# AshHarvey/ssa-gym

Measured on AMD Instinct MI355X. Metric: env_steps_per_sec_at_20k_objects, higher is better.
Workload: dtype f64

## Files before the change

### ssa-gym_amd/csrc/ssa_kernels.hip

```cpp
#include <hip/hip_runtime.h>
#include <cstdio>
#include <cstddef>
#include <cstdlib>
#include <hip/hip_ext.h>
#include <stdint.h>
#include <type_traits>

#include "../../include/ssa_hip.h"
#include "ssa_math.hpp"
#include "ssa_conics.hpp"
#include "ssa_screen.hpp"

namespace ssa {

__device__ __noinline__ Vec6 kepler_general_v(Vec6 x, double tof)
{
    Vec6 o;
    kepler_general_impl(x.v, tof, o.v, nullptr);
    return o;
}
template <int TAG>
__device__ __noinline__ Vec6 kepler_general_tagged(Vec6 x, double tof)
{
    Vec6 o;
// ... 225 lines not shown
        v = sqrt_fast(t.P[g * 36 + 7 * off] + t.P[g * 36 + 7 * (off + 1)] + t.P[g * 36 + 7 * (off + 2)]);
    }
    return v;
}
SSA_DEV void observe_rows(Tiles& t, int g, int l, bool stage_obs)
{
    if (stage_obs && l < 12) t.Obs[g * 12 + l] = (l < 6) ? t.X[g * 6 + l] : t.P[g * 36 + 7 * (l - 6)];
    if (l < 4) t.Met[g * 4 + l] = metric_value(t, g, l);
}

struct Moments { double c00, c01, c11; };
template <bool SUMS_ONLY = false>
SSA_DEV Moments moment_sums_mfma(Tiles& t, int lane)
{
    const int hi = lane >> 4, mid = (lane >> 2) & 3, lo = lane & 3;
    const double* src = &t.D[dbase(mid) + hi * 8 + lo];
    double a0[3], a1[3];
#pragma unroll
    for (int kc = 0; kc < 3; ++kc) {
        a0[kc] = src[kc * 32];
        a1[kc] = src[kc * 32 + 4];
    }
    Moments mo = {0.0, 0.0, 0.0};
#pragma unroll
    for (int kc = 0; kc < 3; ++kc) {
        if (!SUMS_ONLY) mo.c00 = __builtin_amdgcn_mfma_f64_4x4x4f64(a0[kc], a0[kc], mo.c00, 0, 0, 0);
        mo.c01 = __builtin_amdgcn_mfma_f64_4x4x4f64(a0[kc], a1[kc], mo.c01, 0, 0, 0);
        mo.c11 = __builtin_amdgcn_mfma_f64_4x4x4f64(a1[kc], a1[kc], mo.c11, 0, 0, 0);
    }
    if (lo == 2) {
        t.M[mid * 12 + hi] = mo.c01;
        if (hi < 2) t.M[mid * 12 + 4 + hi] = mo.c11;
    }
    return mo;
}

SSA_DEV double covariance_entry(const ssa_consts& C, double acc, double sa_, double ma, double sb_, double mb, double q)
{
    return C.Wi * acc - ma * sb_ - sa_ * mb + C.sum_wc * ma * mb + q;
}
SSA_DEV void covariance_finish(Tiles& t, const ssa_consts& C, int lane, const Moments& mo)
{
    const int hi = lane >> 4, mid = (lane >> 2) & 3, lo = lane & 3;
    const int hi1 = hi & 1, lo1 = lo & 1;
    const double* M = &t.M[mid * 12];
    double* P = &t.P[mid * 36];
    const double s_a = M[hi], m_a = M[6 + hi], s_b = M[lo], m_b = M[6 + lo];
    const double s_a4 = M[4 + hi1], m_a4 = M[10 + hi1], s_b4 = M[4 + lo1], m_b4 = M[10 + lo1];
    const double p00 = covariance_entry(C, mo.c00, s_a, m_a, s_b, m_b, t.Q[hi * 6 + lo]);
    const double p01 = covariance_entry(C, mo.c01, s_a, m_a, s_b4, m_b4, t.Q[hi * 6 + 4 + lo1]);
    const double p11 = covariance_entry(C, mo.c11, s_a4, m_a4, s_b4, m_b4, t.Q[(4 + hi1) * 6 + 4 + lo1]);
    if (hi <= lo) {
        P[hi * 6 + lo] = p00;
        P[lo * 6 + hi] = p00;
    }
    if (lo < 2) {
        P[hi * 6 + 4 + lo] = p01;
        P[(4 + lo) * 6 + hi] = p01;
        if (hi <= lo) {
            P[(4 + hi) * 6 + 4 + lo] = p11;
            P[(4 + lo) * 6 + 4 + hi] = p11;
        }
    }
}

struct StatAcc {
    double mx, sm;
    long long arg;
    unsigned c4, c7, nf;
    int mx_nan, sm_nan;
};
SSA_DEV void stat_merge(StatAcc& a, const StatAcc& b)
{
    a.mx = fmax(a.mx, b.mx);
    a.mx_nan |= b.mx_nan;
    a.c4 += b.c4; a.c7 += b.c7; a.nf += b.nf;
    bool take_b;
    if (a.sm_nan || b.sm_nan) take_b = b.sm_nan && (!a.sm_nan || b.arg < a.arg);
    else take_b = (b.sm > a.sm) || (b.sm == a.sm && b.arg < a.arg);
    if (take_b) { a.sm = b.sm; a.arg = b.arg; a.sm_nan = b.sm_nan; }
}
SSA_DEV StatAcc stat_shfl_down(const StatAcc& a, int off)
{
    StatAcc b;
    b.mx = __shfl_down(a.mx, off, 64);
    b.sm = __shfl_down(a.sm, off, 64);
    b.arg = __shfl_down(a.arg, off, 64);
    b.c4 = __shfl_down(a.c4, off, 64);
    b.c7 = __shfl_down(a.c7, off, 64);
    b.nf = __shfl_down(a.nf, off, 64);
    b.mx_nan = __shfl_down(a.mx_nan, off, 64);
    b.sm_nan = __shfl_down(a.sm_nan, off, 64);
    return b;
}
SSA_DEV StatAcc stat_identity()
{
    StatAcc a;
    a.mx = -1.0; a.sm = -1.0; a.arg = 0x7fffffffffffffffLL; a.c4 = a.c7 = a.nf = 0; a.mx_nan = a.sm_nan = 0;
    return a;
}
SSA_DEV StatAcc stat_wave_reduce(StatAcc a)
{
#pragma unroll
    for (int off = 32; off > 0; off >>= 1) {
        StatAcc b = stat_shfl_down(a, off);
        stat_merge(a, b);
    }
    return a;
}

SSA_DEV void wave_lds_sync()
{
    __builtin_amdgcn_fence(__ATOMIC_ACQ_REL, "wavefront");
    __builtin_amdgcn_wave_barrier();
    asm volatile("" ::: "memory");
}

SSA_DEV int ybase(int g) { return g * 104 + (g & 1) * 28 + (g >> 1) * 32; }
SSA_DEV void covariance_reference(Tiles& t, const ssa_consts& C, int lane, const double (&o)[6], double xb_l)
{
    static_assert(372 + 16 * 8 <= OBJ_PER_WAVE * 36 + 408, "y rows fit the factor tile + D");
    typedef double v2d_t __attribute__((ext_vector_type(2)));
    double* const Y = t.UA;
    {
        const int g = lane >> 4, l = lane & 15;
        const double x0 = row_bcast<0>(xb_l), x1 = row_bcast<1>(xb_l), x2 = row_bcast<2>(xb_l), x3 = row_bcast<3>(xb_l),
                     x4 = row_bcast<4>(xb_l), x5 = row_bcast<5>(xb_l);
        if (l <= 12) {
            v2d_t* dst = reinterpret_cast<v2d_t*>(&Y[ybase(g) + l * 8]);
            dst[0] = v2d_t{o[0] - x0, o[1] - x1};
            dst[1] = v2d_t{o[2] - x2, o[3] - x3};
            dst[2] = v2d_t{o[4] - x4, o[5] - x5};
            dst[3] = v2d_t{0.0, 0.0};
        }
    }
    wave_lds_sync();
    const int hi = lane >> 4, mid = (lane >> 2) & 3, lo = lane & 3;
    const double* src = &Y[ybase(mid) + hi * 8 + lo];
    Moments mo = {0.0, 0.0, 0.0};
    constexpr int NKC = 3;
#pragma unroll
    for (int kc = 0; kc < NKC; ++kc) {
        double a0 = src[kc * 32], a1 = src[kc * 32 + 4];
        if (kc == 3 && hi != 0) { a0 = 0.0; a1 = 0.0; }
        const double w = (kc == 0 && hi == 0) ? C.Wc0 : C.Wi;
        const double b0 = w * a0, b1 = w * a1;
        mo.c00 = __builtin_amdgcn_mfma_f64_4x4x4f64(a0, b0, mo.c00, 0, 0, 0);
        mo.c01 = __builtin_amdgcn_mfma_f64_4x4x4f64(a0, b1, mo.c01, 0, 0, 0);
        mo.c11 = __builtin_amdgcn_mfma_f64_4x4x4f64(a1, b1, mo.c11, 0, 0, 0);
    }
    {
        const double* y12 = &Y[ybase(mid) + 12 * 8];
        const double ai = y12[hi], ai4 = y12[4 + hi], bj = C.Wi * y12[lo], bj4 = C.Wi * y12[4 + lo];
        mo.c00 = fma(ai, bj, mo.c00);
        mo.c01 = fma(ai, bj4, mo.c01);
        mo.c11 = fma(ai4, bj4, mo.c11);
    }
    const int hi1 = hi & 1, lo1 = lo & 1;
    double* P = &t.P[mid * 36];
    const double p00 = mo.c00 + t.Q[hi * 6 + lo];
    const double p01 = mo.c01 + t.Q[hi * 6 + 4 + lo1];
    const double p11 = mo.c11 + t.Q[(4 + hi1) * 6 + 4 + lo1];
    if (hi <= lo) {
        P[hi * 6 + lo] = p00;
        P[lo * 6 + hi] = p00;
    }
    if (lo < 2) {
        P[hi * 6 + 4 + lo] = p01;
        P[(4 + lo) * 6 + hi] = p01;
        if (hi <= lo) {
            P[(4 + hi) * 6 + 4 + lo] = p11;
            P[(4 + lo) * 6 + 4 + hi] = p11;
        }
    }
}

template <int J>
SSA_DEV void chol_step(const double (&a)[6], double (&uc)[6], int lc, bool& ok)
{
    double v = a[J];
#pragma unroll
    for (int i = 0; i < J; ++i) {
        const double uij = row_bcast<J>(uc[i]);
        v = fma(-uij, uc[i], v);
    }
    const double y = row_bcast<J>(rsqrt_nr(v));
    if (J == 5) ok = ok && (y > 0.0) && (y <= 1.79769313486231570e308);
    uc[J] = (lc >= J) ? v * y : 0.0;
}
SSA_DEV double scaled_entry(double scale, double pv, double jit)
{
    double sp = scale * pv;
    SSA_OPAQUE(sp);
    return sp + jit;
}
template <bool PLAIN>
SSA_DEV bool chol_row_regs(const double* Pg, double scale, double jit, int grow, int l, double (&uc)[6])
{
    const int lc = l < 6 ? l : 5;
    double a[6];
    bool ok = true;
#pragma unroll
    for (int j = 0; j < 6; ++j) {
        const double pv = Pg[j * 6 + lc];
        ok = ok && (fabs(pv) <= 1.79769313486231570e308);
        a[j] = (PLAIN || lc != j) ? scale * pv : scaled_entry(scale, pv, jit);
    }
    ok = ((__ballot(!ok) >> (grow * 16)) & 0xFFFFull) == 0;
    chol_step<0>(a, uc, lc, ok);
    chol_step<1>(a, uc, lc, ok);
    chol_step<2>(a, uc, lc, ok);
    chol_step<3>(a, uc, lc, ok);
    chol_step<4>(a, uc, lc, ok);
    chol_step<5>(a, uc, lc, ok);
    return ok;
}
SSA_DEV void chol_store_rows(double* Ug, const double (&uc)[6], int l)
{
    if (l < 6) {
#pragma unroll
        for (int j = 0; j < 6; ++j) Ug[j * 6 + l] = uc[j];
    }
}

__constant__ double JITTER[16] = {1e-6, 1e-5, 1e-4, 1e-3, 1e-2, 1e-1, 1.0, 10.0, 100.0, 1e3, 1e4, 1e5, 1e6, 1e7, 1e8, 1e9};
SSA_DEV bool chol_lane_ok(const double* Pg, double scale, double jit)
{
    double U[21];
    double y = 0.0;
#pragma unroll
    for (int J = 0; J < 6; ++J) {
        double vp = scaled_entry(scale, Pg[J * 6 + J], jit);
#pragma unroll
        for (int i = 0; i < J; ++i) vp = fma(-U[tri(i, J)], U[tri(i, J)], vp);
        y = rsqrt_nr(vp);
#pragma unroll
        for (int c = J + 1; c < 6; ++c) {
            double v = scale * Pg[J * 6 + c];
#pragma unroll
            for (int i = 0; i < J; ++i) v = fma(-U[tri(i, J)], U[tri(i, c)], v);
            U[tri(J, c)] = v * y;
        }
    }
    return (y > 0.0) && (y <= 1.79769313486231570e308);
}
SSA_DEV int robust_chol_row_lds(Tiles& t, double scale, int g, int l)
{
    double uc[6];
    int rung = 16;
    const bool ok = chol_row_regs<true>(&t.P[g * 36], scale, 0.0, g, l, uc);
    if (ok) {
        chol_store_rows(&t.UA[g * 36], uc, l);
        rung = -1;
    }
    const unsigned long long bad = __ballot(!ok);
    wave_lds_sync();
    if (bad == 0ull) return rung;
    __builtin_amdgcn_s_setprio(3);
    const bool mine = ((bad >> (g * 16)) & 1ull) != 0ull;
    if (mine) {
        const double* Pg = &t.P[g * 36];
        const double jit = JITTER[l];
        bool finite = true;
#pragma unroll
        for (int r = 0; r < 3; ++r) {
            const int idx = l + 16 * r;
            if (idx < 36) finite = finite && (fabs(Pg[idx]) <= 1.79769313486231570e308);
        }
        finite = ((__ballot(!finite) >> (g * 16)) & 0xFFFFull) == 0ull;
        const bool okr = chol_lane_ok(Pg, scale, jit) && finite;
        const unsigned won = (unsigned)((__ballot(okr) >> (g * 16)) & 0xFFFFull);
        if (won != 0u) {
            rung = __ffs((int)won) - 1;
            const double jw = __shfl(jit, g * 16 + rung, 64);
            chol_row_regs<false>(Pg, scale, jw, g, l, uc);
            chol_store_rows(&t.UA[g * 36], uc, l);
        }
    }
    wave_lds_sync();
    return rung;
}

SSA_DEV int inline_word(const int32_t (&w)[SSA_INLINE_ENVS], int e)
{
    int v = w[0];
#pragma unroll
    for (int i = 1; i < SSA_INLINE_ENVS; ++i) v = (e == i) ? w[i] : v;
    return v;
}
template <class T> using ConstPtr = const __attribute__((address_space(4))) T*;
typedef const __attribute__((address_space(1))) int32_t* GlobalWords;
typedef int v4i __attribute__((ext_vector_type(4)));
SSA_DEV ConstPtr<ssa_step_params> tile_kernel_params();
template <bool TIME>
SSA_DEV ConstPtr<int32_t> segment_word_src(uint32_t m, const int32_t* mem)
{
    const ConstPtr<ssa_step_params> seg = tile_kernel_params();
    if (TIME) return (m & SSA_LAUNCH_INLINE_ENVS) ? seg->inline_time : (ConstPtr<int32_t>)mem;
    return (m & SSA_LAUNCH_INLINE_ENVS) ? seg->inline_action : (m & SSA_LAUNCH_INLINE_ACTION) ? &seg->action0 : (ConstPtr<int32_t>)mem;
}
SSA_DEV int segment_lane_word(ConstPtr<int32_t> src, int e)
{
    int w = ((GlobalWords)src)[e];
    asm volatile("" : "+v"(w));
    return w;
}
// ... 738 lines not shown
        if constexpr (ENVS) t0 = t_src[asrc.env];
        if constexpr (LENVS) t0 = t_src[asrc.env];
        if (!ALL && !SENS) a0 = *a_src;
        if (hw.obj_ids) {
            const v4i w = *(ConstPtr<v4i>)(hw.obj_ids + base);
            id0 = w.x; id1 = w.y; id2 = w.z; id3 = w.w;
        }
        asm volatile("" : "+s"(t0), "+s"(a0), "+s"(id0), "+s"(id1), "+s"(id2), "+s"(id3));
        if (!ENVS && !LENVS && hw.n_env > 1) {
            t0 = segment_lane_word(t_src, e);
            if (!ALL && !SENS) a0 = segment_lane_word(a_src, e);
        }
        act = valid ? a0 : -1;
        tix = valid ? t0 + hw.time_offset : 0;
    } else if (ALL) {
        act = -1;
        if constexpr (FCAST && LENVS) tix = valid ? asrc.time_word(hw.mask, hw.env_time) + p.time_offset : 0;
        else tix = valid ? env_time_of<INL>(p, e) + p.time_offset : 0;
    } else if (SENS) {
        act = -1;
        if constexpr (ENVS) tix = valid ? env_time_of<INL>(p, asrc.env) + p.time_offset : 0;
        else tix = valid ? env_time_of<INL>(p, 0) + p.time_offset : 0;
    } else if (p.n_env > 1) {
        act = valid ? env_action<INL>(p, e) : -1;
        tix = valid ? env_time_of<INL>(p, e) + p.time_offset : 0;
    } else {
        const int a0 = env_action<INL>(p, 0), t0 = env_time_of<INL>(p, 0);
        act = valid ? a0 : -1;
        tix = valid ? t0 + p.time_offset : 0;
    }
    const bool interval_ok = (hw.update_interval <= 1) || (tix % hw.update_interval == 0);
    int64_t jid = j;
    if (hw.obj_ids) {
        int4 ids;
        if (TILE == 0) ids = make_int4(id0, id1, id2, id3);
        else ids = *reinterpret_cast<const int4*>(hw.obj_ids + base);
        const int mine = (g == 0) ? ids.x : (g == 1) ? ids.y : (g == 2) ? ids.z : ids.w;
        jid = valid ? (int64_t)mine : 0;
        if (l == 0) t.Oid[g] = mine;
    }
    int sid = -1;
    if constexpr (SENS) {
        sid = valid ? sensor_index(asrc, asrc.sites(), jid) : -1;
        act = (sid >= 0) ? (int)jid : -1;
    }
    bool my_update = ALL ? (valid && interval_ok) : SENS ? (sid >= 0 && interval_ok)
                                                         : (!ACT::late && valid && act >= 0 && (int64_t)act == jid && interval_ok);
    const bool may_update = ACT::late ? (valid && interval_ok) : my_update;
    if (!ACT::late && !ALL && __any(my_update)) __builtin_amdgcn_s_setprio(3);
    int tmod = 0;
    double upd_in = 0.0;
    if (may_update && l < ((ALL || DRY) ? 9 : 12)) {
        tmod = time_row(tix, p.n_time);
        const int64_t aobj = ACT::late ? jid : (int64_t)act;
        const double* src = (l < 9) ? p.trans + (int64_t)tmod * 9 + l
                                    : p.z_noise + (int64_t)e * p.zn_stride_env + (int64_t)tmod * p.zn_stride_time + aobj * p.zn_stride_obj + (l - 9);
        if constexpr (SENS) {
            if (l >= 9) src += (int64_t)sid * asrc.sites()->zn_stride_sensor;
        }
        upd_in = *src;
    }

    if (TILE == 0 && pf.dma) tile_dma_wait(t, pf, lane);
    else if (TILE != 2) tile_commit(t, pf, lane);
    if (lane < 8) t.Z[lane] = 0.0;
    if (TILE == 0) {
        if (lane < 36) t.Q[lane] = q_in;
    } else if (TILE != 2 && lane < 36) t.Q[lane] = C.Q[lane];
    wave_lds_sync();

    const int st_in = t.St[g];
    const bool active = valid && st_in == SSA_ST_OK;

    const int rung = robust_chol_row_lds(t, C.scale, g, l);
    asrc.mid_step(t, lane);
    if (may_update && l < 12) t.Obs[g * 12 + l] = upd_in;
    wave_lds_sync();
    const bool chol_fail = (rung == 16);
    const bool is_sigma = (l <= 12);
    const bool is_pm = (l >= 1 && l <= 12);
    double s[6];
    {
        const int krow = (l >= 7) ? l - 7 : l - 1;
        const double sgn = (l >= 7) ? -1.0 : 1.0;
        const bool use_filter = active && !chol_fail && l != 13;
        const double* base = use_filter ? &t.X[g * 6] : &t.T[g * 6];
        const double* urow = (use_filter && is_pm) ? &t.UA[g * 36 + krow * 6] : &t.Z[0];
#pragma unroll
        for (int c = 0; c < 6; ++c) s[c] = fma(sgn, urow[c], base[c]);
    }
    double o[6];
    {
        bool kep_ok;
        if (PROP == 2) {
            const J2Params jq = {C.j2, C.r_eq, C.rk4_substeps};
            kep_ok = propagate_j2_rk4(s, C.dt, jq, o);
        } else {
            if (PROP == 3) kep_ok = kepler_hybrid_fast(s, C.dt, o);
            else kep_ok = kepler_step_fast<PROP == 2 ? 1 : PROP, 1>(s, C.dt, o);
        }
        if (PROP == 3) {
            if (__any(!kep_ok)) {
                bool served = kep_ok;
                if (!ACT::late) {
                    if (!kep_ok) served = kepler_conic_lean<1, true>(s, C.dt, o);
                }
                if (__any(!served)) {
                    __builtin_amdgcn_s_setprio(3);
                    if (!served) {
                        Vec6 si;
#pragma unroll
                        for (int c = 0; c < 6; ++c) si.v[c] = s[c];
                        Vec6 oo = kepler_beyond_series_tagged<1>(si, C.dt);
#pragma unroll
                        for (int c = 0; c < 6; ++c) o[c] = oo.v[c];
                    }
                }
            }
        } else if (PROP != 0) {
            if (__any(!kep_ok)) {
                asm volatile("");
                if (!kep_ok) {
#pragma unroll
                    for (int c = 0; c < 6; ++c) o[c] = __builtin_nan("");
                }
            }
        } else if (__any(!kep_ok)) {
            bool served = kep_ok;
            if (!ACT::late) {
                if (!kep_ok) served = kepler_conic_lean<2, true>(s, C.dt, o);
            }
            if (__any(!served)) {
                if (!served) {
                    Vec6 si;
#pragma unroll
                    for (int c = 0; c < 6; ++c) si.v[c] = s[c];
                    Vec6 oo = kepler_beyond_series_tagged<2>(si, C.dt);
#pragma unroll
                    for (int c = 0; c < 6; ++c) o[c] = oo.v[c];
                }
            }
        }
    }
    wave_lds_sync();
    asm volatile("" : "+v"(lane));
    g = lane >> 4;
    l = lane & 15;
    obj = base + g;
    e = (valid && SSA_NENV > 1) ? (int)((uint32_t)obj / (uint32_t)p.n_obj) : 0;
    if constexpr (ENVS) e = asrc.env;
    if constexpr (FCAST && LENVS) e = asrc.env;
    if (TILE == 1 && !ISSUE_LAST) tile_issue(pf, p, lane, next_base, next_cnt);

    {
        typedef double v2d_t __attribute__((ext_vector_type(2)));
        double d[6];
#pragma unroll
        for (int c = 0; c < 6; ++c) d[c] = o[c] - row_bcast<0>(o[c]);
        if (is_pm) {
            v2d_t* dst = reinterpret_cast<v2d_t*>(&t.D[dbase(g) + (l - 1) * 8]);
            dst[0] = v2d_t{d[0], d[1]};
            dst[1] = v2d_t{d[2], d[3]};
            dst[2] = v2d_t{d[4], d[5]};
            dst[3] = v2d_t{1.0, 0.0};
        } else if (l == 0 || l == 13) {
            v2d_t* dst = reinterpret_cast<v2d_t*>(l == 0 ? &t.X[g * 6] : &t.T[g * 6]);
            dst[0] = v2d_t{o[0], o[1]};
            dst[1] = v2d_t{o[2], o[3]};
            dst[2] = v2d_t{o[4], o[5]};
        }
    }
    wave_lds_sync();
    Moments mo = {0.0, 0.0, 0.0};
    if (C.flags & SSA_FLAG_REFERENCE_COV) mo = moment_sums_mfma<true>(t, lane);
    else mo = moment_sums_mfma(t, lane);
    wave_lds_sync();
    double xb_l = 0.0;
    if (l < 6) {
        const double s0 = t.X[g * 6 + l];
        const double ssum = C.Wi * t.M[g * 12 + l];
        const double mp = C.sum_wm_m1 * s0 + ssum;
        xb_l = s0 + mp;
        t.M[g * 12 + l] = ssum;
        t.M[g * 12 + 6 + l] = mp;
        t.X[g * 6 + l] = xb_l;
    }
    const bool nan_x = ((__ballot(l < 6 && xb_l != xb_l) >> (g * 16)) & 0xFFFFull) != 0;
    wave_lds_sync();
    if (C.flags & SSA_FLAG_REFERENCE_COV) covariance_reference(t, C, lane, o, xb_l);
    else covariance_finish(t, C, lane, mo);
    wave_lds_sync();

    int st_new = st_in;
    if (active) {
        if (chol_fail) st_new = SSA_ST_PREDICT_LINALG;
        else if (nan_x) st_new = SSA_ST_PREDICT_NAN;
    }
    if (!PLAIN && (C.flags & SSA_FLAG_RESAMPLE)) {
        const int rg = robust_chol_row_lds(t, C.scale, g, l);
        wave_lds_sync();
        if (active && st_new == SSA_ST_OK && rg == 16) st_new = SSA_ST_PREDICT_LINALG;
    }
    const int st_pred = st_new;

    if (ACT::late) {
        asrc.before_wait(t, lane, cnt);
        act = asrc.get();
        my_update = valid && act >= 0 && (int64_t)act == (p.obj_ids ? (int64_t)t.Oid[g] : obj) && interval_ok;
        if (__any(my_update)) __builtin_amdgcn_s_setprio(3);
    }
    int look_s = 0;
look_pass:
    if constexpr (LSENS) st_new = st_pred;
    bool look_vis = false, look_taken = false;
    const ssa_sensor_params* SP = PASS_ARGS ? kernarg_opaque(asrc.sites()) : asrc.sites();
    if constexpr (ENVS) sid = valid ? sensor_index(asrc, SP, p.obj_ids ? (int64_t)t.Oid[g] : obj - (int64_t)asrc.env * p.n_obj) : -1;
    else if constexpr (SENS) sid = valid ? sensor_index(asrc, SP, p.obj_ids ? (int64_t)t.Oid[g] : obj) : -1;
    if (__any(my_update)) {
    bool upd_go = false, taken = false, visible = false, attempted = false;
    double z[3] = {0.0, 0.0, 0.0}, y_row[3] = {0.0, 0.0, 0.0};
    double* rec = nullptr;
    double* const STG = &t.UA[g * 117];
    double* const W = &t.D[330];
    static_assert(offsetof(Tiles, D) == offsetof(Tiles, UA) + sizeof(double) * OBJ_PER_WAVE * 36, "UA and D contiguous");
    static_assert(4 * 117 <= OBJ_PER_WAVE * 36 + 330 && 330 + 57 <= 408, "update staging fits");
    if (my_update) {
        if constexpr (SENS) rec = asrc.records(SP) ? asrc.records(SP) + (int64_t)sid * SSA_UPD_STRIDE : nullptr;
        else rec = (!ALL && p.upd) ? p.upd + (int64_t)e * SSA_UPD_STRIDE : nullptr;
        attempted = (st_new == SSA_ST_OK);
        if (attempted) {
            const double* M = &t.Obs[g * 12];
            double sf[6], xb[6];
#pragma unroll
            for (int c = 0; c < 6; ++c) {
                sf[c] = o[c];
                xb[c] = t.X[g * 6 + c];
            }
            if (!PLAIN && (C.flags & SSA_FLAG_RESAMPLE) && (!LSENS || look_s == 0)) {
                const int krow = is_pm ? (l - 1) % 6 : 0;
                const double sgn = (l >= 1 && l <= 6) ? 1.0 : ((l >= 7 && l <= 12) ? -1.0 : 0.0);
#pragma unroll
                for (int c = 0; c < 6; ++c)
                    if (l != 13) sf[c] = xb[c] + sgn * t.UA[g * 36 + krow * 6 + c];
            }
            if constexpr (LSENS) {
                if (look_s == 0) {
                    if (l <= 12) {
#pragma unroll
                        for (int c = 0; c < 6; ++c) STG[l * 9 + c] = sf[c];
                    }
                } else {
#pragma unroll
                    for (int c = 0; c < 6; ++c) sf[c] = (l <= 12) ? STG[l * 9 + c] : t.T[g * 6 + c];
                }
            } else if (l <= 12) {
#pragma unroll
                for (int c = 0; c < 6; ++c) STG[l * 9 + c] = sf[c] - xb[c];
            }
            double enu_vec[3];
            double el_mine;
            double lim = 0.0;
            {
                double Mm[9], aer[3];
#pragma unroll
                for (int i = 0; i < 9; ++i) Mm[i] = M[i];
                if constexpr (SENS) {
                    for (;;) {
                        const int su = __builtin_amdgcn_readfirstlane(sid);
                        if (sid == su) {
                            hx_aer_enu(sf, Mm, SP->enu[su], SP->obs_itrs[su], aer, enu_vec);
                            lim = SP->obs_limit[su];
                            break;
                        }
                    }
                } else if constexpr (LSENS) {
                    hx_aer_enu(sf, Mm, SP->enu[look_s], SP->obs_itrs[look_s], aer, enu_vec);
                    lim = SP->obs_limit[look_s];
                } else hx_aer_enu(sf, Mm, C.enu, C.obs_itrs, aer, enu_vec);
                el_mine = aer[1];
                if (PLAIN || C.obs_type == SSA_OBS_AER) { z[0] = aer[0]; z[1] = aer[1]; z[2] = aer[2]; }
                else { z[0] = sf[0]; z[1] = sf[1]; z[2] = sf[2]; }
            }
            if constexpr (SENS || LSENS) visible = row_bcast<13>(el_mine) >= lim;
            else visible = row_bcast<13>(el_mine) >= C.obs_limit;
            if (rec && l == 13) {
#pragma unroll
                for (int c = 0; c < 3; ++c) rec[SSA_UPD_Z_TRUE + c] = z[c];
            }
            if (visible) {
                double zp[3];
                const double wl = (l == 0) ? C.Wc0 : (is_pm ? C.Wi : 0.0);
                if (PLAIN || C.obs_type == SSA_OBS_AER) {
                    double um[3];
#pragma unroll
                    for (int c = 0; c < 3; ++c) {
                        double u0 = row_bcast<0>(enu_vec[c]);
                        double du = is_pm ? (enu_vec[c] - u0) : 0.0;
                        um[c] = u0 + (C.sum_wm_m1 * u0 + C.Wi * row_allsum(du));
                    }
                    uvw2aer(um, zp);
                } else {
#pragma unroll
                    for (int c = 0; c < 3; ++c) {
                        double u0 = row_bcast<0>(z[c]);
                        double du = is_pm ? (z[c] - u0) : 0.0;
                        zp[c] = u0 + (C.sum_wm_m1 * u0 + C.Wi * row_allsum(du));
                    }
                }
                double rz[3];
                {
                    double zin[3];
                    if (l == 13) {
                        const double* zn = &t.Obs[g * 12 + 9];
#pragma unroll
                        for (int c = 0; c < 3; ++c) zin[c] = z[c] + zn[c];
                    } else {
#pragma unroll
                        for (int c = 0; c < 3; ++c) zin[c] = z[c];
                    }
                    if (PLAIN || C.obs_type == SSA_OBS_AER) residual_z_aer_wrapped(zin, zp, rz);
                    else {
#pragma unroll
                        for (int c = 0; c < 3; ++c) rz[c] = zin[c] - zp[c];
                    }
                }
                if constexpr (SENS) {
                    if ((SP->angles_only >> sid) & 1) rz[2] = 0.0;
                } else if constexpr (LSENS) {
                    if ((SP->angles_only >> look_s) & 1) rz[2] = 0.0;
                }
                upd_go = true;
                if (l <= 12) {
#pragma unroll
                    for (int c = 0; c < 3; ++c) STG[l * 9 + 6 + c] = rz[c];
                }
                if (l == 13) {
#pragma unroll
                    for (int c = 0; c < 3; ++c) y_row[c] = rz[c];
                }
            }
        }
    }
// ... 3513 lines not shown
```

Measured before the change: 79350.

## Store raw sigma-point rows in LDS for reference-covariance predict path

For the PLAIN kernel variant with the reference-covariance flag, the predict step now writes the raw propagated sigma points into the factor tile region instead of differences from the mean sigma point. It then computes the mean sums with an MFMA reduction against a one-hot vector, and builds the covariance with MFMA from rows centered on the updated mean. This replaces the per-lane covariance_reference path with tensor-core products. It adds LDS layout aliasing (sbase into UA), which brings a risk of overlap, and it only applies when the reference-covariance flag is set.

```diff
diff --git a/ssa-gym_amd/csrc/ssa_kernels.hip b/ssa-gym_amd/csrc/ssa_kernels.hip
--- a/ssa-gym_amd/csrc/ssa_kernels.hip
+++ b/ssa-gym_amd/csrc/ssa_kernels.hip
@@ -401,6 +401,98 @@
     {
         const double* y12 = &Y[ybase(mid) + 12 * 8];
         const double ai = y12[hi], ai4 = y12[4 + hi], bj = C.Wi * y12[lo], bj4 = C.Wi * y12[4 + lo];
+        mo.c00 = fma(ai, bj, mo.c00);
+        mo.c01 = fma(ai, bj4, mo.c01);
+        mo.c11 = fma(ai4, bj4, mo.c11);
+    }
+    const int hi1 = hi & 1, lo1 = lo & 1;
+    double* P = &t.P[mid * 36];
+    const double p00 = mo.c00 + t.Q[hi * 6 + lo];
+    const double p01 = mo.c01 + t.Q[hi * 6 + 4 + lo1];
+    const double p11 = mo.c11 + t.Q[(4 + hi1) * 6 + 4 + lo1];
+    if (hi <= lo) {
+        P[hi * 6 + lo] = p00;
+        P[lo * 6 + hi] = p00;
+    }
+    if (lo < 2) {
+        P[hi * 6 + 4 + lo] = p01;
+        P[(4 + lo) * 6 + hi] = p01;
+        if (hi <= lo) {
+            P[(4 + hi) * 6 + 4 + lo] = p11;
+            P[(4 + lo) * 6 + 4 + hi] = p11;
+        }
+    }
+}
+
+SSA_DEV int sbase(int g) { return g * 104 + (g & 1) * 28 + (g >> 1) * 32; }
+static_assert(372 + 13 * 8 <= OBJ_PER_WAVE * 36 + 408, "the rows of sigma points fit the factor tile + D");
+SSA_DEV void sigma_rows_write(Tiles& t, int g, int l, const double (&o)[6])
+{
+    typedef double v2d_t __attribute__((ext_vector_type(2)));
+    if (l <= 12) {
+        v2d_t* dst = reinterpret_cast<v2d_t*>(&t.UA[sbase(g) + l * 8]);
+        dst[0] = v2d_t{o[0], o[1]};
+        dst[1] = v2d_t{o[2], o[3]};
+        dst[2] = v2d_t{o[4], o[5]};
+    }
+    if (l == 0 || l == 13) {
+        v2d_t* dst = reinterpret_cast<v2d_t*>(l == 0 ? &t.X[g * 6] : &t.T[g * 6]);
+        dst[0] = v2d_t{o[0], o[1]};
+        dst[1] = v2d_t{o[2], o[3]};
+        dst[2] = v2d_t{o[4], o[5]};
+    }
+}
+SSA_DEV void moment_sums_rows(Tiles& t, int lane)
+{
+    const int hi = lane >> 4, mid = (lane >> 2) & 3, lo = lane & 3;
+    const double* src = &t.UA[sbase(mid) + hi * 8 + lo];
+    const double* s0 = &t.UA[sbase(mid) + lo];
+    const double z0 = s0[0], z1 = s0[4];
+    double a0[3], a1[3];
+#pragma unroll
+    for (int kc = 0; kc < 3; ++kc) {
+        a0[kc] = src[8 + kc * 32];
+        a1[kc] = src[8 + kc * 32 + 4];
+    }
+    const double one = (lo == 2) ? 1.0 : 0.0;
+    double c01 = 0.0, c11 = 0.0;
+#pragma unroll
+    for (int kc = 0; kc < 3; ++kc) {
+        const double d0 = a0[kc] - z0, d1 = a1[kc] - z1;
+        c01 = __builtin_amdgcn_mfma_f64_4x4x4f64(d0, one, c01, 0, 0, 0);
+        c11 = __builtin_amdgcn_mfma_f64_4x4x4f64(d1, one, c11, 0, 0, 0);
+    }
+    if (lo == 2) {
+        t.M[mid * 12 + hi] = c01;
+        if (hi < 2) t.M[mid * 12 + 4 + hi] = c11;
+    }
+}
+SSA_DEV void covariance_reference_rows(Tiles& t, const ssa_consts& C, int lane)
+{
+    const int hi = lane >> 4, mid = (lane >> 2) & 3, lo = lane & 3;
+    const double* src = &t.UA[sbase(mid) + hi * 8 + lo];
+    const double* r12 = &t.UA[sbase(mid) + 12 * 8];
+    const double* xb = &t.X[mid * 6];
+    double a0[3], a1[3];
+#pragma unroll
+    for (int kc = 0; kc < 3; ++kc) {
+        a0[kc] = src[kc * 32];
+        a1[kc] = src[kc * 32 + 4];
+    }
+    const double x_lo = xb[lo], x_lo4 = xb[4 + lo], x_hi = xb[hi], x_hi4 = xb[4 + hi];
+    const double s_lo = r12[lo], s_lo4 = r12[4 + lo], s_hi = r12[hi], s_hi4 = r12[4 + hi];
+    Moments mo = {0.0, 0.0, 0.0};
+#pragma unroll
+    for (int kc = 0; kc < 3; ++kc) {
+        const double y0 = a0[kc] - x_lo, y1 = a1[kc] - x_lo4;
+        const double w = (kc == 0 && hi == 0) ? C.Wc0 : C.Wi;
+        const double b0 = w * y0, b1 = w * y1;
+        mo.c00 = __builtin_amdgcn_mfma_f64_4x4x4f64(y0, b0, mo.c00, 0, 0, 0);
+        mo.c01 = __builtin_amdgcn_mfma_f64_4x4x4f64(y0, b1, mo.c01, 0, 0, 0);
+        mo.c11 = __builtin_amdgcn_mfma_f64_4x4x4f64(y1, b1, mo.c11, 0, 0, 0);
+    }
+    {
+        const double ai = s_hi - x_hi, ai4 = s_hi4 - x_hi4, bj = C.Wi * (s_lo - x_lo), bj4 = C.Wi * (s_lo4 - x_lo4);
         mo.c00 = fma(ai, bj, mo.c00);
         mo.c01 = fma(ai, bj4, mo.c01);
         mo.c11 = fma(ai4, bj4, mo.c11);
@@ -1445,7 +1537,10 @@
     if constexpr (FCAST && LENVS) e = asrc.env;
     if (TILE == 1 && !ISSUE_LAST) tile_issue(pf, p, lane, next_base, next_cnt);
 
-    {
+    const bool rows_form = PLAIN && (C.flags & SSA_FLAG_REFERENCE_COV);
+    if (rows_form) {
+        sigma_rows_write(t, g, l, o);
+    } else {
         typedef double v2d_t __attribute__((ext_vector_type(2)));
         double d[6];
 #pragma unroll
@@ -1465,7 +1560,8 @@
     }
     wave_lds_sync();
     Moments mo = {0.0, 0.0, 0.0};
-    if (C.flags & SSA_FLAG_REFERENCE_COV) mo = moment_sums_mfma<true>(t, lane);
+    if (rows_form) moment_sums_rows(t, lane);
+    else if (!PLAIN && (C.flags & SSA_FLAG_REFERENCE_COV)) mo = moment_sums_mfma<true>(t, lane);
     else mo = moment_sums_mfma(t, lane);
     wave_lds_sync();
     double xb_l = 0.0;
@@ -1480,7 +1576,8 @@
     }
     const bool nan_x = ((__ballot(l < 6 && xb_l != xb_l) >> (g * 16)) & 0xFFFFull) != 0;
     wave_lds_sync();
-    if (C.flags & SSA_FLAG_REFERENCE_COV) covariance_reference(t, C, lane, o, xb_l);
+    if (rows_form) covariance_reference_rows(t, C, lane);
+    else if (!PLAIN && (C.flags & SSA_FLAG_REFERENCE_COV)) covariance_reference(t, C, lane, o, xb_l);
     else covariance_finish(t, C, lane, mo);
     wave_lds_sync();
 
```

New measurement: 81830, median of 6. +3.1%, better.
